# pymc-devs/pymc

Measured on AMD Instinct MI355X. Metric: effective samples/sec (and leapfrog steps/sec), 10k-param hierarchical logistic regression, one NUTS chain per GPU, higher is better.
Workload: dtype f64

## Files before the change

include/nuts_mi355.h:

```cpp
#ifndef NUTS_MI355_H
#define NUTS_MI355_H

#include <stdint.h>

#ifdef __cplusplus
extern "C" {
#endif

#define NUTS_OK 0
#define NUTS_E_BAD_ENERGY 1
#define NUTS_E_ARG 2
#define NUTS_E_HIP 3
#define NUTS_E_LINALG 4
#define NUTS_E_CALLBACK 5


enum { NUTS_TR_NONE = 0, NUTS_TR_LOG = 1, NUTS_TR_LOGODDS = 2, NUTS_TR_INTERVAL = 3 };
enum {
  NUTS_OP_CONST = 0, NUTS_OP_DATA = 1, NUTS_OP_VAR = 2,
  NUTS_OP_TMP = 3,
  NUTS_OP_GATHER = 4,
  NUTS_OP_LIN = 5
};
enum {
// ... 122 lines not shown
  const double *glm_X;
  const double *glm_y;
  int32_t n_lins, pad3;
  const nuts_lin *lins;
} nuts_model_spec;
enum { NUTS_GLM_NORMAL = 0, NUTS_GLM_BERNOULLI = 1, NUTS_GLM_POISSON = 2 };
#define NUTS_GLM_MAXP 512

typedef struct nuts_model nuts_model;
typedef struct nuts_chain nuts_chain;

int nuts_set_option(const char *name, int32_t value);
int nuts_unset_option(const char *name);
void nuts_clear_options(void);

int nuts_device_count(void);
int nuts_set_device(int device);
const char *nuts_last_error(void);

nuts_model *nuts_model_create(const nuts_model_spec *spec);
void nuts_model_destroy(nuts_model *m);
int32_t nuts_model_ndim(const nuts_model *m);
int nuts_model_logp_grad(nuts_model *m, const double *q, double *logp, double *grad);
int nuts_model_time_logp_grad(nuts_model *m, const double *q, int reps, double *ms_total, double *ms_dominant);
int nuts_model_debug_ticks(nuts_model *m, int64_t *out );
int64_t nuts_model_algorithmic_bytes(const nuts_model *m);
int nuts_model_get_scalar(const nuts_model *m, const char *name, double *out);

enum { NUTS_POT_DIAG_ADAPT = 0, NUTS_POT_DIAG = 1, NUTS_POT_FULL = 2,
       NUTS_POT_DIAG_ADAPT_EXP = 3,
// ... 168 lines not shown
```

pymc_amd/_lib.py:

```python

from __future__ import annotations

import ctypes as C
import os
import threading

import numpy as np

_HERE = os.path.dirname(os.path.abspath(__file__))
LIB_PATH = os.path.join(_HERE, "libnuts_mi355.so")

NUTS_OK, NUTS_E_BAD_ENERGY, NUTS_E_ARG, NUTS_E_HIP, NUTS_E_LINALG, NUTS_E_CALLBACK = 0, 1, 2, 3, 4, 5


class EngineError(RuntimeError):
    """A HIP/runtime failure inside libnuts_mi355 (maps to ParallelSamplingError-style reporting)."""


class Operand(C.Structure):
    _fields_ = [("kind", C.c_int32), ("ref", C.c_int32), ("c", C.c_double)]


class Term(C.Structure):
    _fields_ = [("a", Operand), ("b", Operand), ("c", Operand)]
# ... 222 lines not shown
    "nuts_chain_set_log_step_bar": (C.c_int, [_VP, C.c_double, C.c_double]),
    "nuts_gibbs_plan": (C.c_int, [C.POINTER(Pcg64), C.c_int64, C.c_int32, _VP, _VP, _VP, _PD]),
    "nuts_gibbs_plan_shuffle": (C.c_int, [C.POINTER(Pcg64), C.c_int64, _VP]),
    "nuts_gibbs_plan_draws": (C.c_int, [C.POINTER(Pcg64), C.c_int64, _VP, _VP, _VP, _PD, C.POINTER(C.c_int32)]),
    "nuts_gibbs_plan_skip": (C.c_int, [C.POINTER(Pcg64), C.c_int64, C.c_int32]),
    "nuts_gibbs_create": (_VP, [C.c_int64, C.c_int32, _PD]),
    "nuts_gibbs_destroy": (None, [_VP]),
    "nuts_gibbs_stage_slots": (C.c_int, []),
    "nuts_gibbs_stage": (C.c_int, [_VP, C.c_int32, _VP, _VP, _PD]),
    "nuts_gibbs_sweep_staged": (C.c_int, [_VP, C.c_int32, _VP, _VP, C.c_int32, _PD, _PD, _PD, C.POINTER(C.c_int64), C.POINTER(C.c_int64), _PD, _PD, _PD]),
    "nuts_gibbs_sweep": (C.c_int, [_VP, _VP, _PD, _PD, _PD, _VP, _VP, _PD, C.POINTER(C.c_int64), C.POINTER(C.c_int64), _PD, _PD, _PD]),
    "nuts_gibbs_plan_doubles": (C.c_int, [C.POINTER(Pcg64), C.c_int64, C.c_int32, _VP, C.c_int64, _PD]),
    "nuts_gibbs_sweep_prop": (C.c_int, [_VP, _VP, _VP, _PD, _PD, _PD, _VP, _PD, _PD, _VP, C.POINTER(C.c_int64), _PD, _PD, _PD]),
    "nuts_set_option": (C.c_int, [C.c_char_p, C.c_int32]),
    "nuts_clear_options": (None, []),
    "nuts_advi_create": (_VP, [C.POINTER(AdviConfig)]),
    "nuts_advi_destroy": (None, [_VP]),
    "nuts_advi_steps": (C.c_int, [_VP, C.c_int32, _VP, _PD, _PD]),
    "nuts_advi_get_params": (C.c_int, [_VP, _PD, _PD]),
    "nuts_advi_set_params": (C.c_int, [_VP, _PD, _PD]),
    "nuts_chain_profile": (C.c_int, [_VP, C.c_int]),
    "nuts_chain_profile_read": (C.c_int, [_VP, _PD, C.POINTER(C.c_int64), C.POINTER(C.c_int64)]),
    "nuts_group_create": (_VP, []),
    "nuts_group_add": (C.c_int, [_VP, _VP]),
    "nuts_group_remove": (C.c_int, [_VP, _VP]),
    "nuts_group_destroy": (None, [_VP]),
    "nuts_group_launches": (C.c_int, [_VP, C.POINTER(C.c_int64)]),
    "nuts_group_launches_wide": (C.c_int, [_VP, C.POINTER(C.c_int64), C.POINTER(C.c_int32)]),
    "nuts_unset_option": (C.c_int, [C.c_char_p]),
}
# ... 102 lines not shown
```

pymc_amd/csrc/engine.hip:

```cpp
#include <hip/hip_runtime.h>

#include <algorithm>
#include <atomic>
#include <chrono>
#include <cmath>
#include <cstdio>
#include <cstdlib>
#include <cstring>
#include <mutex>
#include <thread>
#include <utility>
#include <ctime>
#include <string>
#include <vector>

#include "kernels.h"
#include "small_kernel.h"
#include "mixture_kernel.h"
#include "nuts_mi355.h"
#include "pcg64_stream.h"
#include "advi.h"

static thread_local std::string g_err;

// ... 29 lines not shown
}

template <typename T>
static T* dev_alloc(size_t count) {
  void* p = nullptr;
  const size_t bytes = std::max<size_t>(count, 1) * sizeof(T);
  if (hipMalloc(&p, bytes) != hipSuccess) return nullptr;
  if (env_int("NUTS_POISON_ALLOC", 0)) { hipMemset(p, 0xFF, bytes); hipDeviceSynchronize(); }
  return static_cast<T*>(p);
}
template <typename T>
static T* dev_upload(const T* src, size_t count) {
  T* p = dev_alloc<T>(count);
  if (p && count) hipMemcpy(p, src, count * sizeof(T), hipMemcpyHostToDevice);
  return p;
}

#define PROF_RUN_MIN 16
#define SMALL_MAX_ELEMS 16384
#define SMALL_MAX_N 1024

struct nuts_model {
  ModelDev md{};
  hipStream_t stream = nullptr;
  std::vector<void*> owned;
  double* q_dev = nullptr;
  double* g_dev = nullptr;
  double* lp_dev = nullptr;
  double* host_pin = nullptr;
  std::vector<nuts_data_ref> data_refs;
// ... 13 lines not shown
  std::vector<int32_t> ev_units;
  int run_open = 0;
  int64_t runs_seen = 0;
  size_t ev_used = 0;
  int64_t dom_launches = 0;
  int sample_every = 1;
  hipStream_t own_stream = nullptr;
  struct nuts_group* group = nullptr;
  bool g_active = false;
  int gslot = 0;
  int n_chains = 0;
  int64_t pool_extra = 0;
  int64_t orphan_elems = 0, factor_elems = 0;
  double rows_pack_s = 0.0;
  int64_t rows_xt_len = 0, rows_y_len = 0;
  std::vector<LinDev> lins_host;

  template <typename T>
  T* keep(T* p) {
    owned.push_back((void*)p);
    return p;
  }
};

extern "C" int nuts_device_count(void) {
  int n = 0;
  if (hipGetDeviceCount(&n) != hipSuccess) return 0;
  return n;
}
extern "C" int nuts_set_device(int device) {
// ... 352 lines not shown
    if (prof) { hipEventRecord(m->ev[m->ev_used + 1], m->stream); m->ev_used += 2; m->dom_units += 1; }
    m->dom_launches++;
    hipLaunchKernelGGL(k_glm_reduce, dim3((md.glm.Ppad + 3 + GLM_RED_COLS - 1) / GLM_RED_COLS), dim3(GLM_RED_CHUNKS * GLM_RED_COLS), 0, m->stream, md, A, io, j);
    if (!md.has_mvn) return;
    prof = false; m->dom_launches--;
  }
  if (md.has_logit && md.lg.ga) {
    const int rev = m->rows_alternate ? (m->rows_flip ^= 1) : 0;
    const int par = (m->ga_par ^= 1);
    const dim3 grid(m->rows_grid + (fold ? 1 : 0) + md.lg.ga_naux), block(WAVE * md.lg.ga_w);
    GaArgs ga{md, A, io, j, rev, fold ? (GA_FOLD_CTL | GA_FOLD_SRC) : 0, par, d, max_depth, Emax, st, io, j - 1, d, 0, 0};
    if (fold && job) {
      ga.fold = GA_FOLD_CTL | (job->src_prev ? GA_FOLD_SRC : 0);
      ga.cio = job->io; ga.cj = job->j; ga.cd = job->d; ga.cseq = job->seq;
    }
    if (m->group && m->g_active && io.mode == MODE_TREE && m->group->kind >= 2) {
      GaLeafArgs L;
      L.A = A; L.io = io; L.cio = ga.cio; L.Emax = Emax; L.st = st;
      L.ga_part = md.lg.ga_part; L.ga_bpart = md.lg.ga_bpart; L.ga_ticket = md.lg.ga_ticket; L.def_loc = md.def_loc;
      L.j = j; L.fold = ga.fold; L.par = par; L.d = d; L.max_depth = max_depth; L.cj = ga.cj; L.cd = ga.cd; L.cseq = ga.cseq;
      L.slot = m->gslot; L.pad = 0;
      group_deposit(m, L);
    } else
    if (md.lg.ga_gpw) {
      switch (md.lg.D) {
        case 8: if (md.lg.ga_dx == 7) hipLaunchKernelGGL((k_rows_gb<8, 7>), grid, block, 0, m->stream, ga);
                else hipLaunchKernelGGL((k_rows_gb<8>), grid, block, 0, m->stream, ga); break;
        case 4: hipLaunchKernelGGL((k_rows_gb<4>), grid, block, 0, m->stream, ga); break;
        case 2: hipLaunchKernelGGL((k_rows_gb<2>), grid, block, 0, m->stream, ga); break;
        case 1: hipLaunchKernelGGL((k_rows_gb<1>), grid, block, 0, m->stream, ga); break;
// ... 799 lines not shown
      lg.Xp = m->keep(dev_upload(xp.data(), xp.size()));
      lg.ga_pcoff = m->keep(dev_upload(pcoff.data(), pcoff.size()));
      lg.ga_pexc_idx = m->keep(dev_upload(exc_idx.data(), exc_idx.size()));
      lg.ga_pexc = m->keep(dev_upload(exc.data(), exc.size()));
      lg.ga_pack_ebase20 = (uint32_t)plan.elo << 20;
      lg.ga_pack = (lg.Xp && lg.ga_pcoff && lg.ga_pexc_idx && lg.ga_pexc) ? 1 : 0;
      if (!lg.ga_pack) (void)hipGetLastError();
    }
    m->rows_pack_s = std::chrono::duration<double>(std::chrono::steady_clock::now() - t0).count();
  }
  lg.ga_coff = m->keep(dev_upload(coff.data(), coff.size()));
  lg.ga_tile0 = m->keep(dev_upload(tile0.data(), tile0.size()));
  lg.ga_part = m->keep(dev_alloc<double>((size_t)lg.G * PART_STRIDE));
  const size_t bpart_len = gpw ? 2 * (size_t)PART_STRIDE * ((lg.ga_nrec + WAVE - 1) / WAVE * WAVE) : 2 * (size_t)lg.ga_nrec * PART_STRIDE;
  lg.ga_bpart = m->keep(dev_alloc<double>(bpart_len));
  lg.ga_ticket = m->keep(dev_alloc<unsigned>(lg.ga_nblk));
  if (lg.ga_part) hipMemset(lg.ga_part, 0, (size_t)lg.G * PART_STRIDE * sizeof(double));
  if (lg.ga_bpart) hipMemset(lg.ga_bpart, 0, bpart_len * sizeof(double));
  if (lg.ga_ticket) hipMemset(lg.ga_ticket, 0, lg.ga_nblk * sizeof(unsigned));
  m->rows_grid = gpw ? lg.ga_nblk : lg.G;
  return true;
}

static bool build_rows_spans(nuts_model* m, const nuts_model_spec* s, int cus) {
  RowsDev& lg = m->md.lg;
  const int D = lg.D, SPAN = WAVE * m->rows_rpl;
  const int32_t* gid = s->rows_gid;
  int wpc = env_int("NUTS_ROWS_WAVES_PER_CU", 0);
  if (wpc <= 0) {
    const int64_t spans = (s->rows_N + (int64_t)WAVE * m->rows_rpl - 1) / ((int64_t)WAVE * m->rows_rpl);
    wpc = spans >= (int64_t)cus * 32 * 4 ? 32 : 16;
  }
  {
    std::vector<double> xt((size_t)D * lg.Npad, 0.0);
// ... 460 lines not shown
extern "C" int nuts_model_debug_ticks(nuts_model* m, int64_t* out) {
  if (!m || !out) return NUTS_E_ARG;
  HIPCHK(hipStreamSynchronize(m->stream));
  HIPCHK(hipMemcpy(out, m->md.ticks, 64 * sizeof(long long), hipMemcpyDeviceToHost));
  return NUTS_OK;
}

extern "C" int32_t nuts_model_ndim(const nuts_model* m) { return m ? m->md.n : -1; }
extern "C" int nuts_model_get_scalar(const nuts_model* m, const char* name, double* out) {
  if (!m || !name || !out) return NUTS_E_ARG;
  const std::string k(name);
  if (k == "rows_group_aligned") *out = m->md.lg.ga;
  else if (k == "rows_group_block") *out = m->md.lg.ga_gpw;
  else if (k == "rows_packed") *out = m->md.lg.ga ? m->md.lg.ga_pack : 0;
  else if (k == "rows_pack_build_s") *out = m->rows_pack_s;
  else if (k == "rows_aux_workgroups") *out = m->md.lg.ga ? m->md.lg.ga_naux : 0;
  else if (k == "mixture_workgroups") *out = m->md.has_mix ? m->md.mix.nwg : 0;
  else if (k == "glm_workgroups") *out = m->md.has_glm ? m->md.glm.nwg : 0;
  else if (k == "glm_row_stride") *out = m->md.has_glm ? m->md.glm.xstride : 0;
  else if (k == "glm_layout_width") *out = m->md.has_glm ? m->md.glm.Ppad : 0;
  else if (k == "mvn_row_aligned") *out = m->md.has_mvn ? m->md.mv.aligned : 0;
  else if (k == "rows_waves") *out = m->md.lg.ga ? m->md.lg.ga_w : m->md.lg.n_waves;
  else if (k == "lean") *out = m->md.lean_ok;
  else if (k == "chain_group_kind") {
    const RowsDev& lg = m->md.lg;
    const bool is_mvn = m->md.has_mvn && (m->md.mv.aligned == 4 || m->md.mv.aligned == 8 || m->md.mv.aligned == 16);
    const bool is_rows = m->md.has_logit && !m->md.has_mvn && lg.ga && lg.ga_naux == 0 && lg.D == 8 && m->ga_struct_ok == 1;
    *out = is_mvn ? 1.0 : (is_rows ? (lg.ga_gpw > 0 ? 3.0 : 2.0) : 0.0);
  }
  else if (k == "chain_group_wide_ok") *out = (m->md.has_mvn && m->md.mv.aligned > 0 && m->md.mv.k % 16 == 0) ? 1.0 : 0.0;
// ... 176 lines not shown
  std::vector<double> div_source, div_dest;
  bool cache_ok = false;
  std::vector<double> last_q;
  double last_logp = 0.0;
  DrawOut* do_dev = nullptr;
  DrawOut* do_host = nullptr;
  DrawOutMapped* dom_host = nullptr;
  DrawOutMapped* dom_dev = nullptr;
  unsigned dom_seq = 0;
  double* kin_part = nullptr;
  int64_t cache_epoch = -1;
  int fold_ctl = 1;
  CtlJob pend{}; bool pend_valid = false;
  bool defer_last_ctl = false; int xfold = 1;
  int next_dir = 0; bool pre_done = false; int xpre = 1;
  int spec_max = 10, last_depth = 0;
  int pipe_draws = 1;
  int logs_done = 0, logs_total = 0;
  double* many_in_host = nullptr; double* many_in_dev = nullptr; char* many_out_host = nullptr; char* many_out_dev = nullptr;
  size_t many_in_cap = 0, many_out_cap = 0;
  double t_begin = 0, t_loop = 0, t_wait = 0, t_finish = 0, t_post = 0;
  double tm_pre = 0, tm_start = 0, tm_tree = 0, tm_record = 0, tm_host = 0, tm_post = 0;
  int64_t tm_draws = 0, tm_batches = 0;
  int64_t leapfrogs = 0;
  int n_uni_cap = 0;
  template <typename T>
  T* keep(T* p) { owned.push_back((void*)p); return p; }
};

extern "C" void nuts_chain_config_default(nuts_chain_config* c) {
// ... 134 lines not shown
  A.S = 1 << maxd;
  A.ept = m->ept;
  A.nblk = m->md.nblk;
  const size_t arena = (size_t)A.S * n;
  A.Q = c->keep(dev_alloc<double>(arena)); A.P = c->keep(dev_alloc<double>(arena));
  A.V = c->keep(dev_alloc<double>(arena)); A.G = c->keep(dev_alloc<double>(arena));
  A.E = c->keep(dev_alloc<double>(A.S)); A.LOGP = c->keep(dev_alloc<double>(A.S));
  A.PS = c->keep(dev_alloc<double>((size_t)MAX_LEVELS * n));
  A.PSUM = c->keep(dev_alloc<double>(n));
  c->kin_part = c->keep(dev_alloc<double>((size_t)A.nblk));
  A.ctl = c->keep(dev_alloc<Ctl>(1));
  c->var = c->keep(dev_alloc<double>(n)); c->stds = c->keep(dev_alloc<double>(n)); c->inv_stds = c->keep(dev_alloc<double>(n));
  c->wa_mean = c->keep(dev_alloc<double>(n)); c->wa_m2 = c->keep(dev_alloc<double>(n));
  c->wb_mean = c->keep(dev_alloc<double>(n)); c->wb_m2 = c->keep(dev_alloc<double>(n));
  A.var = c->var; A.inv_stds = c->inv_stds;
  A.ga_ticket = m->md.lg.ga ? m->md.lg.ga_ticket : nullptr; A.ga_nticket = m->md.lg.ga ? m->md.lg.ga_nblk : 0;
  if (c->full_adapt) {
    const size_t nn = (size_t)n * n;
    c->fa_initial_cov.assign(cfg->dense_cov, cfg->dense_cov + nn);
    c->dense_C = c->keep(dev_alloc<double>(nn));
    c->fa_L = c->keep(dev_alloc<double>(nn)); c->fa_Lw = c->keep(dev_alloc<double>(nn));
    c->fa_fg_raw = c->keep(dev_alloc<double>(nn)); c->fa_bg_raw = c->keep(dev_alloc<double>(nn));
    c->fa_fg_mean = c->keep(dev_alloc<double>(n)); c->fa_bg_mean = c->keep(dev_alloc<double>(n));
    c->fa_scratch = c->keep(dev_alloc<double>(4 * (size_t)n)); c->fa_rhs = c->keep(dev_alloc<double>(n));
    c->fa_fail = c->keep(dev_alloc<int>(2));
    c->mv_grid = (n + (256 / WAVE) - 1) / (256 / WAVE);
  } else if (c->host_pot) {
    c->hp_p.assign(n, 0.0); c->hp_v.assign(n, 0.0);
    c->kin_user_dev = c->keep(dev_alloc<double>(1));
    A.kin_user = c->kin_user_dev;
  } else if (c->dense) {
    c->dense_C = c->keep(dev_upload(cfg->dense_cov, (size_t)n * n));
    c->dense_W = c->keep(dev_upload(cfg->dense_rand, (size_t)n * n));
    c->mv_grid = (n + (256 / WAVE) - 1) / (256 / WAVE);
  }
  c->n_uni_cap = (1 << maxd) + 2 * maxd + 16;
  c->stage_dev = c->keep(dev_alloc<double>(2 * (size_t)n + 2 * (size_t)c->n_uni_cap));
  c->out_dev = c->keep(dev_alloc<double>(2 * (size_t)n));
  c->out_dev2 = c->keep(dev_alloc<double>(2 * (size_t)n + 2));
  c->fold_ctl = env_int("NUTS_FOLD_CTL", 1) != 0 && !(m->md.has_mvn && m->md.mv.winv);
  c->spec_max = env_int("NUTS_SPEC_MAX", 10);
  c->xfold = env_int("NUTS_XFOLD", 1);
  c->pipe_draws = env_int("NUTS_PIPE_DRAWS", 1) != 0;
  c->xpre = env_int("NUTS_XPRE", 1);
  c->small_lds_slots = env_int("NUTS_SMALL_LDS", 1) == 0 ? -1 : env_int("NUTS_SMALL_LDS_SLOTS", 0);
  c->small_one_wave = env_int("NUTS_SMALL_ONE_WAVE", 1);
  c->group_wide = env_int("NUTS_GROUP_WIDE", 0);
  const bool glm_small = m->md.has_glm && env_int("NUTS_GLM_SMALL", 1) != 0 && m->md.glm.Xt && !m->md.glm.beta_buf && m->md.glm.off_beta >= 0 && m->md.n_derived == 0 && n <= 256;
  c->small = env_int("NUTS_SMALL_KERNEL", 1) != 0 && n <= SMALL_MAX_N && m->ept == 1 && !m->md.has_logit && !m->md.has_mvn && !m->md.has_mix &&
             (!m->md.has_glm || glm_small) &&
             m->md.n_lins == 0 && m->factor_elems <= SMALL_MAX_ELEMS && !c->dense;
  c->do_dev = c->keep(dev_alloc<DrawOut>(1));
  A.uniforms = c->stage_dev + 2 * (size_t)n;
  A.log_uniforms = A.uniforms + c->n_uni_cap;
  for (void* p : c->owned)
    if (!p) { g_err = "device allocation failed (trajectory arena needs 4*2^max_treedepth*n*8 bytes)"; nuts_chain_destroy(c); return nullptr; }
  if (hipHostMalloc((void**)&c->stage_host, (2 * (size_t)n + 2 * (size_t)c->n_uni_cap) * sizeof(double), hipHostMallocDefault) != hipSuccess ||
// ... 541 lines not shown
  int rc = NUTS_OK;
  bool exhausted = true;
  GroupTreeScope lockstep(c->dense || c->host_pot ? nullptr : c->m);
  unsigned flags = 0;
  Geometry gm{uniforms[0] < 0.5 ? 1 : -1, 0, 0, 0, 0.0};
  gm.eps = gm.dir > 0 ? step_size : -step_size;
  auto next_geometry = [&](const Geometry& g, int d, int dir) {
    Geometry r = g;
    if (g.dir > 0) r.right += 1 << d; else r.left -= 1 << d;
    r.dir = dir;
    r.edge = dir > 0 ? r.right : r.left;
    r.eps = dir > 0 ? step_size : -step_size;
    return r;
  };
  const int spec = c->host_pot ? 0 : std::min(c->spec_max, c->last_depth - 1);
  auto enqueue_doubling = [&](const Geometry& g, int d) {
    const int nleaf = 1 << d;
    ensure_logs(c, (2 << d) + d + 1);
    const int seq = ++c->seq;
    c->defer_last_ctl = c->xfold && c->fold_ctl && d + 1 < max_depth && d + 1 <= spec;
    c->next_dir = c->defer_last_ctl ? (uniforms[(2 << d) + d] < 0.5 ? 1 : -1) : 0;
    for (int j = 0; j < nleaf; ++j) enqueue_leaf(c, g, j, d, MODE_TREE, max_depth, j + 1 == nleaf ? seq : 0);
    c->defer_last_ctl = false;
    return seq;
  };
  c->pre_done = false;
  c->pend_valid = false;
  auto flush_pending = [&](int seq_waited) {
    if (!c->pend_valid || c->pend.seq != seq_waited) return;
    const CtlJob& p = c->pend;
    launch_control_lean(c->m, c->A, p.io, p.j, p.d, c->cfg.Emax, max_depth, c->st_dev, p.seq);
    c->pend_valid = false;
  };
  Geometry ahead{};
  int ahead_seq = 0;
  int seq = enqueue_doubling(gm, 0);
  int depth_done = 0;
// ... 1 lines not shown
    if (d + 1 < max_depth && d + 1 <= spec) {
      ahead = next_geometry(gm, d, uniforms[(2 << d) + d] < 0.5 ? 1 : -1);
      ahead_seq = enqueue_doubling(ahead, d + 1);
    } else ahead_seq = 0;
    flush_pending(seq);
    if (c->cb_err) return host_pot_error(c);
    const auto tw0 = clk::now();
    rc = wait_status(c, seq, &flags, cursor_out);
    c->t_wait += secs(tw0, clk::now());
    if (rc) return rc;
    depth_done = d + 1;
    if (flags & ST_BAD_ENERGY) break;
    if (flags & (ST_DIVERGING | ST_TURNING)) { exhausted = false; break; }
    if (d + 1 >= max_depth) break;
    const int dir = (flags & ST_DIR_POS) ? 1 : -1;
    if (ahead_seq) {
      if (ahead.dir != dir) { g_err = "internal error: look-ahead mispredicted the direction of a doubling"; return NUTS_E_HIP; }
      gm = ahead; seq = ahead_seq;
    } else {
      gm = next_geometry(gm, d, dir);
      seq = enqueue_doubling(gm, d + 1);
    }
  }
  c->last_depth = depth_done;
  c->pend_valid = false;
  *flags_out = flags;
  *exhausted_out = exhausted;
  return NUTS_OK;
}

static void launch_small(nuts_chain* c, const ArenaDev& A, const SmallDrawArgs& a) {
#define SMALL_LAUNCH(NT, P) hipLaunchKernelGGL((k_small_draw<NT, P>), dim3(1), dim3(NT), 0, c->m->stream, c->m->md, A, a)
  const bool hp = c->m->has_prog;
  if (c->n <= WAVE && c->small_one_wave && !c->m->md.has_glm) { if (hp) SMALL_LAUNCH(64, true); else SMALL_LAUNCH(64, false); }
  else if (c->n <= 256) { if (hp) SMALL_LAUNCH(256, true); else SMALL_LAUNCH(256, false); }
  else if (c->n <= 512) { if (hp) SMALL_LAUNCH(512, true); else SMALL_LAUNCH(512, false); }
  else { if (hp) SMALL_LAUNCH(1024, true); else SMALL_LAUNCH(1024, false); }
#undef SMALL_LAUNCH
}

// ... 1123 lines not shown
```

pymc_amd/csrc/rows_ga_kernel.h:

```cpp
#pragma once
#include "rows_kernel.h"
#include "rows_pack.h"

__device__ __forceinline__ void ga_def_local(const RowsDev& R, bool is_mu, double qn, double& gx, double& dxdq, double& dj, double& lp) {
  if (is_mu) {
    const double r = qn - R.mu_c[0];
    const double z = r * R.mu_c[1];
    lp = -0.5 * z * z - R.mu_c[2] + (-0.91893853320467274178);
    gx = -z * R.mu_c[1]; dxdq = 1.0; dj = 0.0;
  } else {
    double x, lj;
    if (R.sigma_tr == NUTS_TR_LOG) { x = exp(qn); dxdq = x; lj = qn; dj = 1.0; }
    else { x = qn; dxdq = 1.0; lj = 0.0; dj = 0.0; }
    const double z = x * R.sg_c[0];
    double lpf = -0.5 * z * z - R.sg_c[1] + (-0.22579135264472743236);
    double g = -z * R.sg_c[0];
    if (!(x >= 0)) { lpf = -INFINITY; g = 0.0; }
    gx = g; lp = lj + lpf;
  }
}

template <int D, int RPL>
__device__ __forceinline__ void ga_load(const RowsDev& R, int64_t xoff, int lane, double (&x)[D][RPL], uint32_t& ybits) {
  constexpr int SPAN = WAVE * RPL;
// ... 186 lines not shown
    for (int d = 0; d < D; ++d) eta = fma(x[d][k], beta[d], eta);
    double l, rr;
    logit_row(eta, (double)((yb >> (8 * k)) & 0xffu), l, rr);
    const bool in = lane * RPL + k < nvalid;
    lp += in ? l : 0.0;
    rr = in ? rr : 0.0;
#pragma unroll
    for (int d = 0; d < D; ++d) acc[d] = fma(rr, x[d][k], acc[d]);
    if constexpr (!ILV) __builtin_amdgcn_sched_barrier(0);
  }
}

#define GA_MAXW 4
#define GA_MAXCHUNK 8
#define GA_F_NOTAIL 1

struct GaArgs;
template <int D>
__device__ __forceinline__ void ga_tail(const GaArgs& T, int g, double (&s_acc)[4][2][D + 1], double (&s_red)[NDOT],
                                        double (&s_cp)[8][PART_STRIDE], int (&s_info)[4], double (&s_keep)[5][WAVE]);

struct GaArgs {
  ModelDev md; ArenaDev A; EvalIO io;
  int j, rev, fold, par, d, max_depth;
  double Emax;
  HostStatus* st;
  EvalIO cio;
  int cj, cd, cseq, cpad;
};
#define GA_FOLD_CTL 1
// ... 352 lines not shown
  const bool tree = io.mode == MODE_TREE;
  const int dl = lane % D;
  const int iz = R.off_z + g * D + dl;
  MergePrefetch mpf;
  if (w == 0 && tree && !(R.ga_flags & GA_F_NOTAIL)) merge_prefetch(A, lf, j, iz, mpf);
  __syncthreads();
  if (R.ga_flags & GA_F_NOTAIL) return;

  if (w == 0)
    ga_tail_wave<D, false>(R, A, io, R.ga_part, R.ga_ticket, md.def_loc, lf, g, W, j, T.par, T.d, s_acc, s_red, s_info,
                           s_keep[0][lane], s_keep[1][lane], s_keep[2][lane], s_keep[3][lane], s_keep[4][lane], &mpf);
  __syncthreads();
  if (!s_info[0]) return;
  ga_block_partial<D>(R, R.ga_part, R.ga_bpart, T.par, g, leaf, s_info, s_cp);
}
```

pymc_amd/csrc/rows_ga_multi_kernel.h:

```cpp
#pragma once
#include "mvn_multi_kernel.h"

#define GAM_MAXC 8
#define GAM_MAXNC 4

struct GaLeafArgs {
  ArenaDev A;
  EvalIO io, cio;
  double Emax;
  HostStatus* st;
  double* ga_part;
  double* ga_bpart;
  unsigned* ga_ticket;
  double* def_loc;
  int j, fold, par, d, max_depth, cj, cd, cseq;
  int slot, pad;
};

template <int NC>
struct GaMultiArgs {
  GaLeafArgs c[NC];
  int rev, pad;
};

__device__ __forceinline__ LeanSrc gam_src(const RowsDev& R, const GaLeafArgs& L, int par) {
  return LeanSrc{L.ga_bpart + (int64_t)par * R.ga_nrec * PART_STRIDE, PART_STRIDE, R.ga_nrec, L.def_loc + (int64_t)par * 4 * MAX_DEFERRED};
}

template <int DX>
__device__ __forceinline__ void gam_load(const double* base , const int8_t* ybase, int lane,
                                         typename GaTileSel<DX>::type& t) {
  const ga_v2d* p = reinterpret_cast<const ga_v2d*>(base) + lane;
#pragma unroll
  for (int k = 0; k < DX; ++k) t.c[k] = p[k * WAVE];
  t.y = *reinterpret_cast<const uint16_t*>(ybase + 2 * lane);
}

template <int NC, int OCC, int DX>
__global__ __launch_bounds__(64 * GA_MAXW, OCC) void k_rows_ga_multi(ModelDev md, GaMultiArgs<NC> ma) {
  constexpr int D = 8, RPL = 2, SPAN = WAVE * RPL, PIPE = 2;
  typedef typename GaTileSel<DX>::type Tile;
  const RowsDev& R = md.lg;
  if ((int)blockIdx.x < GAM_MAXC) {
    int ci = -1;
#pragma unroll
    for (int c = 0; c < NC; ++c) ci = (int)blockIdx.x == ma.c[c].slot ? c : ci;
    if (ci < 0) return;
    const GaLeafArgs& L = ma.c[ci];
    if (L.fold & GA_FOLD_CTL) control_lean(md, L.A, L.cio, L.cj, L.cd, L.Emax, L.max_depth, L.st, L.cseq, gam_src(R, L, L.par ^ 1));
    return;
  }
  const int g = (int)blockIdx.x - GAM_MAXC;
  const int rev = ma.rev;
  const int tid = threadIdx.x, lane = tid & (WAVE - 1), w = __builtin_amdgcn_readfirstlane(tid >> 6), W = (int)blockDim.x >> 6;
  __shared__ double s_acc[NC][GA_MAXW][2][D + 1];
  __shared__ double s_red[NC][NDOT];
  __shared__ double s_cp[GA_MAXCHUNK][PART_STRIDE];
  __shared__ int s_info[NC][4];
  __shared__ double s_keep[NC][5][WAVE];
  __shared__ double s_beta[NC][D];
  __shared__ __attribute__((aligned(16))) char s_args[(sizeof(GaMultiArgs<NC>) + 15) / 16 * 16];

  int T; int64_t ng, cbase;
  if (R.ga_T_uni > 0) { T = R.ga_T_uni; ng = R.ga_ng_uni; cbase = (int64_t)(g * W + w) * R.ga_cstride_uni; }
  else {
    T = __builtin_amdgcn_readfirstlane(R.ga_tile0[g + 1] - R.ga_tile0[g]);
    ng = __builtin_amdgcn_readfirstlane((int)(R.gptr[g + 1] - R.gptr[g]));
    const int64_t cb = R.ga_coff[g * W + w];
    cbase = ((int64_t)__builtin_amdgcn_readfirstlane((int)(cb >> 32)) << 32) | (uint32_t)__builtin_amdgcn_readfirstlane((int)(cb & 0xffffffffll));
  }
  const int c0 = (int)((int64_t)w * T / W), c2 = (int)((int64_t)(w + 1) * T / W);
  const int n = c2 - c0;
  const int nA = (n + 1) / 2;
  const int nsw = rev ? n - nA : nA;
  constexpr int64_t TS = (int64_t)DX * SPAN;
  auto local_at = [&](int i) { return rev ? (i < nsw ? nA + i : i - nsw) : i; };
  auto tile_at = [&](int i) { return cbase + (int64_t)local_at(i) * TS; };
  const int l_last = (c2 == T) ? n - 1 : -1;
  const int n_last = (int)(ng - (int64_t)(T - 1) * SPAN);
  if (lane == 0) {
#pragma unroll
    for (int c = 0; c < NC; ++c)
#pragma unroll
      for (int dd = 0; dd <= D; ++dd) { s_acc[c][w][0][dd] = 0.0; s_acc[c][w][1][dd] = 0.0; }
  }
  {
    static_assert(alignof(GaMultiArgs<NC>) == 8 && sizeof(GaMultiArgs<NC>) % 8 == 0, "kernarg layout: the second argument follows the model at the next multiple of 8");
    const uint2* ka = (const uint2*)__builtin_amdgcn_kernarg_segment_ptr() + (sizeof(ModelDev) + 7) / 8;
    for (int t = tid; t < (int)(sizeof(GaMultiArgs<NC>) / 8); t += (int)blockDim.x) reinterpret_cast<uint2*>(s_args)[t] = ka[t];
  }

  int dead = 0;
#pragma unroll
  for (int c = 0; c < NC; ++c) dead |= load_aborted(ma.c[c].io, ma.c[c].A) ? (1 << c) : 0;
  if (dead == (1 << NC) - 1) return;
  for (int c = w; c < NC; c += W) {
    const GaLeafArgs& L = ma.c[c];
    Leaf lf; QView qv;
    resolve_leaf(L.io, L.A, L.j, lf, qv);
    double hval0, hph0;
    ga_hyper<D>(R, qv, L.fold, gam_src(R, L, L.par ^ 1), lane, hval0, hph0);
    const int dl = lane % D;
    const int iz = R.off_z + g * D + dl;
    double zq, zph, m_lane, s_lane;
    ga_z_state(qv, iz, zq, zph);
    ga_hyper_lanes<D>(R, hval0, dl, m_lane, s_lane);
    const double bl = fma(s_lane, zq, m_lane);
    if (lane < D) s_beta[c][lane] = bl;
    s_keep[c][0][lane] = hval0; s_keep[c][1][lane] = hph0; s_keep[c][2][lane] = zq; s_keep[c][3][lane] = zph; s_keep[c][4][lane] = s_lane;
  }
  __syncthreads();
  constexpr bool TWO = NC <= 3;
  Tile ta, tb;
  {
    const int64_t o0 = tile_at(0), o1 = tile_at(min(1, max(n - 1, 0)));
    gam_load<DX>(R.Xt + o0, R.y + o0 / DX, lane, ta);
// ... 57 lines not shown
        if (i + 1 >= n) break;
        issue(i + 2, ta);
        GAM_STAGE(tb, i + 1)
        issue(i + 3, tb);
      }
    } else {
      for (int i = 0; i < n; ++i) {
        GAM_STAGE(ta, i)
        issue(i + 1, ta);
      }
    }
#undef GAM_STAGE
    if (n > 0) flush();
  }

  const GaMultiArgs<NC>& Tm = *reinterpret_cast<const GaMultiArgs<NC>*>(s_args);
  MergePrefetch mpf;
  if (w < NC && !((dead >> w) & 1)) {
    const GaLeafArgs& L = Tm.c[w];
    Leaf lf; QView qv;
    resolve_leaf(L.io, L.A, L.j, lf, qv);
    merge_prefetch(L.A, lf, L.j, R.off_z + g * D + lane % D, mpf);
  }
  __syncthreads();
  for (int c = w; c < NC; c += W) {
    if ((dead >> c) & 1) { if (lane == 0) s_info[c][0] = 0; continue; }
    const GaLeafArgs& L = Tm.c[c];
    Leaf lf; QView qv;
    resolve_leaf(L.io, L.A, L.j, lf, qv);
    auto tail = [&](const MergePrefetch* pf) {
      ga_tail_wave<D, true>(R, L.A, L.io, L.ga_part, L.ga_ticket, L.def_loc, lf, g, W, L.j, L.par, L.d, s_acc[c], s_red[c], s_info[c],
                            s_keep[c][0][lane], s_keep[c][1][lane], s_keep[c][2][lane], s_keep[c][3][lane], s_keep[c][4][lane], pf);
    };
    if (c == w) tail(&mpf);
    else tail(nullptr);
  }
  __syncthreads();
#pragma unroll
  for (int c = 0; c < NC; ++c) {
    if (!s_info[c][0]) continue;
    ga_block_partial<D>(R, Tm.c[c].ga_part, Tm.c[c].ga_bpart, Tm.c[c].par, g, true, s_info[c], s_cp);
    __syncthreads();
  }
}
// ... 1 lines not shown
```

Baseline: 19160.

## Pair NUTS leaf evaluations with speculative opposite-direction shadow leaves via ring buffer

When the tree is expected to turn, each leaf evaluation also computes a speculative leaf on the opposite trajectory edge inside the same multi-leaf rows kernel. The shadow leaf's per-group partial sums go to a device ring buffer, and a later doubling in that direction replays them through a lighter tail-only kernel instead of streaming the design matrix again. The aim is to amortise X reads across two leaves per pass. The cost is extra ring, partial and shadow-state memory, wasted shadow work when the tree stops early, and more complex ticket and parity bookkeeping.

```diff
diff --git a/include/nuts_mi355.h b/include/nuts_mi355.h
--- a/include/nuts_mi355.h
+++ b/include/nuts_mi355.h
@@ -160,6 +160,9 @@
 int nuts_unset_option(const char *name);
 void nuts_clear_options(void);
 
+int64_t nuts_edge_pair_plan(const int32_t *dirs, int32_t n_dirs, int32_t n_doublings, int32_t spec, int32_t max_depth,
+                            int32_t ring, int32_t *out, int64_t out_cap);
+
 int nuts_device_count(void);
 int nuts_set_device(int device);
 const char *nuts_last_error(void);
diff --git a/pymc_amd/_lib.py b/pymc_amd/_lib.py
--- a/pymc_amd/_lib.py
+++ b/pymc_amd/_lib.py
@@ -260,6 +260,7 @@
     "nuts_gibbs_sweep_prop": (C.c_int, [_VP, _VP, _VP, _PD, _PD, _PD, _VP, _PD, _PD, _VP, C.POINTER(C.c_int64), _PD, _PD, _PD]),
     "nuts_set_option": (C.c_int, [C.c_char_p, C.c_int32]),
     "nuts_clear_options": (None, []),
+    "nuts_edge_pair_plan": (C.c_int64, [C.POINTER(C.c_int32), C.c_int32, C.c_int32, C.c_int32, C.c_int32, C.c_int32, C.POINTER(C.c_int32), C.c_int64]),
     "nuts_advi_create": (_VP, [C.POINTER(AdviConfig)]),
     "nuts_advi_destroy": (None, [_VP]),
     "nuts_advi_steps": (C.c_int, [_VP, C.c_int32, _VP, _PD, _PD]),
diff --git a/pymc_amd/csrc/engine.hip b/pymc_amd/csrc/engine.hip
--- a/pymc_amd/csrc/engine.hip
+++ b/pymc_amd/csrc/engine.hip
@@ -67,6 +67,48 @@
   T* p = dev_alloc<T>(count);
   if (p && count) hipMemcpy(p, src, count * sizeof(T), hipMemcpyHostToDevice);
   return p;
+}
+
+enum { EP_PLAIN = 0, EP_PAIRED = 1, EP_REPLAY = 2 };
+struct EdgePlan {
+  int ring = 64;
+  int side = 0, n = 0;
+  unsigned head = 0;
+  int cap = 0, used = 0;
+  int64_t ring_full = 0;
+  void reset() { side = 0; n = 0; cap = 0; used = 0; }
+  template <class F>
+  void begin(int d, int dir, int last, F dir_of) {
+    cap = 0; used = 0;
+    for (int e = d + 1; e <= last; ++e)
+      if (dir_of(e) == -dir) { cap = std::min(1 << std::min(e, 30), ring); break; }
+  }
+  int leaf(int dir, int* slot, int* k) {
+    if (n > 0 && side == dir) { *slot = (int)(head % (unsigned)ring); *k = used++; ++head; --n; return EP_REPLAY; }
+    if (cap > 0 && n < cap) { side = -dir; *k = n; *slot = (int)((head + (unsigned)n) % (unsigned)ring); ++n; return EP_PAIRED; }
+    if (cap > 0 && n >= ring) ++ring_full;
+    *slot = -1; *k = -1;
+    return EP_PLAIN;
+  }
+};
+extern "C" int64_t nuts_edge_pair_plan(const int32_t* dirs, int32_t n_dirs, int32_t n_doublings, int32_t spec, int32_t max_depth,
+                                       int32_t ring, int32_t* out, int64_t out_cap) {
+  if (!dirs || !out || n_doublings < 0 || n_doublings > n_dirs || n_doublings > 20 || ring < 1) { g_err = "nuts_edge_pair_plan: bad argument"; return -1; }
+  EdgePlan ep;
+  ep.ring = ring;
+  int64_t n = 0;
+  const int last = std::min(std::min(spec, max_depth - 1), n_dirs - 1);
+  for (int d = 0; d < n_doublings; ++d) {
+    ep.begin(d, dirs[d], last, [&](int e) { return (int)dirs[e]; });
+    for (int j = 0; j < (1 << d); ++j, ++n) {
+      int slot, k;
+      const int kind = ep.leaf(dirs[d], &slot, &k);
+      if (n >= out_cap) { g_err = "nuts_edge_pair_plan: output too small"; return -1; }
+      int32_t* o = out + 5 * n;
+      o[0] = d; o[1] = j; o[2] = kind; o[3] = slot; o[4] = k;
+    }
+  }
+  return n;
 }
 
 #define PROF_RUN_MIN 16
@@ -110,6 +152,16 @@
   int64_t orphan_elems = 0, factor_elems = 0;
   double rows_pack_s = 0.0;
   int64_t rows_xt_len = 0, rows_y_len = 0;
+  int ep_ok = 0, ep_par = 0;
+  double *ep_ring = nullptr, *ep_part = nullptr, *ep_bpart = nullptr, *ep_def_loc = nullptr;
+  int64_t ep_ring_bytes = 0, ep_shadows = 0, ep_replays = 0;
+  int64_t ep_dropped = 0;
+  int64_t ep_ring_full = 0;
+  int ep_turns = 0;
+  struct EpLaunch {
+    int kind = EP_PLAIN, slot = 0, sj = 0, sfold = 0, first = 0;
+    EvalIO sio{}; ArenaDev sA{};
+  } ep_launch;
   std::vector<LinDev> lins_host;
 
   template <typename T>
@@ -492,6 +544,32 @@
       ga.fold = GA_FOLD_CTL | (job->src_prev ? GA_FOLD_SRC : 0);
       ga.cio = job->io; ga.cj = job->j; ga.cd = job->d; ga.cseq = job->seq;
     }
+    const nuts_model::EpLaunch ep = m->ep_launch;
+    m->ep_launch.kind = EP_PLAIN;
+    if (ep.kind == EP_PAIRED) {
+      GaMultiArgs<2, true> ma;
+      GaLeafArgs& L = ma.c[0];
+      L.A = A; L.io = io; L.cio = ga.cio; L.Emax = Emax; L.st = st;
+      L.ga_part = md.lg.ga_part; L.ga_bpart = md.lg.ga_bpart; L.ga_ticket = md.lg.ga_ticket; L.def_loc = md.def_loc;
+      L.j = j; L.fold = ga.fold; L.par = par; L.d = d; L.max_depth = max_depth; L.cj = ga.cj; L.cd = ga.cd; L.cseq = ga.cseq;
+      L.slot = 0; L.pad = 0;
+      GaLeafArgs& S = ma.c[1];
+      S.A = ep.sA; S.io = ep.sio; S.cio = ep.sio; S.Emax = Emax; S.st = nullptr;
+      S.ga_part = m->ep_part; S.ga_bpart = m->ep_bpart; S.ga_ticket = md.lg.ga_ticket + md.lg.ga_nblk; S.def_loc = m->ep_def_loc;
+      S.j = ep.sj; S.fold = ep.sfold; S.par = (m->ep_par ^= 1); S.d = 0; S.max_depth = 1; S.cj = 0; S.cd = 0; S.cseq = 0;
+      S.slot = GAM_MAXC - 1; S.pad = ep.first ? GAM_SH_FIRST : 0;
+      ma.rev = rev; ma.pad = 0;
+      ma.ring = m->ep_ring + (size_t)ep.slot * md.lg.G * GA_RING_DOUBLES(8);
+      const dim3 pgrid(GAM_MAXC + md.lg.G);
+      if (md.lg.ga_dx == 7) hipLaunchKernelGGL((k_rows_ga_multi<2, 3, 7, true>), pgrid, block, 0, m->stream, md, ma);
+      else hipLaunchKernelGGL((k_rows_ga_multi<2, 3, 8, true>), pgrid, block, 0, m->stream, md, ma);
+      m->ep_shadows++;
+    } else if (ep.kind == EP_REPLAY) {
+      const dim3 rgrid(m->rows_grid + (fold ? 1 : 0));
+      hipLaunchKernelGGL((k_rows_ga_replay<8>), rgrid, block, 0, m->stream, ga,
+                         (const double*)(m->ep_ring + (size_t)ep.slot * md.lg.G * GA_RING_DOUBLES(8)));
+      m->ep_replays++;
+    } else
     if (m->group && m->g_active && io.mode == MODE_TREE && m->group->kind >= 2) {
       GaLeafArgs L;
       L.A = A; L.io = io; L.cio = ga.cio; L.Emax = Emax; L.st = st;
@@ -1321,10 +1399,24 @@
   lg.ga_part = m->keep(dev_alloc<double>((size_t)lg.G * PART_STRIDE));
   const size_t bpart_len = gpw ? 2 * (size_t)PART_STRIDE * ((lg.ga_nrec + WAVE - 1) / WAVE * WAVE) : 2 * (size_t)lg.ga_nrec * PART_STRIDE;
   lg.ga_bpart = m->keep(dev_alloc<double>(bpart_len));
-  lg.ga_ticket = m->keep(dev_alloc<unsigned>(lg.ga_nblk));
+  lg.ga_ticket = m->keep(dev_alloc<unsigned>(2 * (size_t)lg.ga_nblk));
   if (lg.ga_part) hipMemset(lg.ga_part, 0, (size_t)lg.G * PART_STRIDE * sizeof(double));
   if (lg.ga_bpart) hipMemset(lg.ga_bpart, 0, bpart_len * sizeof(double));
-  if (lg.ga_ticket) hipMemset(lg.ga_ticket, 0, lg.ga_nblk * sizeof(unsigned));
+  if (lg.ga_ticket) hipMemset(lg.ga_ticket, 0, 2 * (size_t)lg.ga_nblk * sizeof(unsigned));
+  m->ep_ok = 0;
+  if (!gpw && D == 8 && m->rows_rpl == 2 && m->ga_struct_ok == 1 && lg.ga_naux == 0 && env_int("NUTS_EDGE_PAIR", 1) != 0) {
+    const size_t ring_len = (size_t)GA_RING_LEAVES * lg.G * GA_RING_DOUBLES(8);
+    m->ep_ring = m->keep(dev_alloc<double>(ring_len));
+    m->ep_part = m->keep(dev_alloc<double>((size_t)lg.G * PART_STRIDE));
+    m->ep_bpart = m->keep(dev_alloc<double>(bpart_len));
+    m->ep_def_loc = m->keep(dev_alloc<double>(2 * 4 * (size_t)MAX_DEFERRED));
+    if (m->ep_ring && m->ep_part && m->ep_bpart && m->ep_def_loc) {
+      hipMemset(m->ep_part, 0, (size_t)lg.G * PART_STRIDE * sizeof(double));
+      hipMemset(m->ep_bpart, 0, bpart_len * sizeof(double));
+      hipMemset(m->ep_def_loc, 0, 2 * 4 * (size_t)MAX_DEFERRED * sizeof(double));
+      m->ep_ok = 1; m->ep_ring_bytes = (int64_t)(ring_len * sizeof(double));
+    } else (void)hipGetLastError();
+  }
   m->rows_grid = gpw ? lg.ga_nblk : lg.G;
   return true;
 }
@@ -1815,6 +1907,13 @@
   else if (k == "rows_group_block") *out = m->md.lg.ga_gpw;
   else if (k == "rows_packed") *out = m->md.lg.ga ? m->md.lg.ga_pack : 0;
   else if (k == "rows_pack_build_s") *out = m->rows_pack_s;
+  else if (k == "edge_pair") *out = m->ep_ok;
+  else if (k == "edge_pair_ring_bytes") *out = (double)m->ep_ring_bytes;
+  else if (k == "edge_pair_shadows") *out = (double)m->ep_shadows;
+  else if (k == "edge_pair_replays") *out = (double)m->ep_replays;
+  else if (k == "edge_pair_turns") *out = m->ep_turns;
+  else if (k == "edge_pair_dropped") *out = (double)m->ep_dropped;
+  else if (k == "edge_pair_ring_full") *out = (double)m->ep_ring_full;
   else if (k == "rows_aux_workgroups") *out = m->md.lg.ga ? m->md.lg.ga_naux : 0;
   else if (k == "mixture_workgroups") *out = m->md.has_mix ? m->md.mix.nwg : 0;
   else if (k == "glm_workgroups") *out = m->md.has_glm ? m->md.glm.nwg : 0;
@@ -2021,6 +2120,9 @@
   CtlJob pend{}; bool pend_valid = false;
   bool defer_last_ctl = false; int xfold = 1;
   int next_dir = 0; bool pre_done = false; int xpre = 1;
+  bool edge_pair = false;
+  ArenaDev shA{};
+  EdgePlan ep;
   int spec_max = 10, last_depth = 0;
   int pipe_draws = 1;
   int logs_done = 0, logs_total = 0;
@@ -2185,7 +2287,7 @@
   c->wa_mean = c->keep(dev_alloc<double>(n)); c->wa_m2 = c->keep(dev_alloc<double>(n));
   c->wb_mean = c->keep(dev_alloc<double>(n)); c->wb_m2 = c->keep(dev_alloc<double>(n));
   A.var = c->var; A.inv_stds = c->inv_stds;
-  A.ga_ticket = m->md.lg.ga ? m->md.lg.ga_ticket : nullptr; A.ga_nticket = m->md.lg.ga ? m->md.lg.ga_nblk : 0;
+  A.ga_ticket = m->md.lg.ga ? m->md.lg.ga_ticket : nullptr; A.ga_nticket = m->md.lg.ga ? 2 * m->md.lg.ga_nblk : 0;
   if (c->full_adapt) {
     const size_t nn = (size_t)n * n;
     c->fa_initial_cov.assign(cfg->dense_cov, cfg->dense_cov + nn);
@@ -2212,6 +2314,16 @@
   c->fold_ctl = env_int("NUTS_FOLD_CTL", 1) != 0 && !(m->md.has_mvn && m->md.mv.winv);
   c->spec_max = env_int("NUTS_SPEC_MAX", 10);
   c->xfold = env_int("NUTS_XFOLD", 1);
+  c->edge_pair = m->ep_ok && env_int("NUTS_EDGE_PAIR", 1) != 0 && !c->dense && !c->host_pot && !m->md.has_mvn && !m->explicit_pre &&
+                 m->md.lean_ok && c->fold_ctl && c->xfold;
+  if (c->edge_pair) {
+    c->shA = A;
+    c->shA.S = 2;
+    c->shA.Q = c->keep(dev_alloc<double>(2 * (size_t)n)); c->shA.P = c->keep(dev_alloc<double>(2 * (size_t)n));
+    c->shA.V = c->keep(dev_alloc<double>(2 * (size_t)n)); c->shA.G = c->keep(dev_alloc<double>(2 * (size_t)n));
+    if (!c->shA.Q || !c->shA.P || !c->shA.V || !c->shA.G) { (void)hipGetLastError(); c->edge_pair = false; }
+    c->ep.ring = std::max(1, std::min(GA_RING_LEAVES, env_int("NUTS_EDGE_PAIR_RING", GA_RING_LEAVES)));
+  }
   c->pipe_draws = env_int("NUTS_PIPE_DRAWS", 1) != 0;
   c->xpre = env_int("NUTS_XPRE", 1);
   c->small_lds_slots = env_int("NUTS_SMALL_LDS", 1) == 0 ? -1 : env_int("NUTS_SMALL_LDS_SLOTS", 0);
@@ -2783,13 +2895,41 @@
     return r;
   };
   const int spec = c->host_pot ? 0 : std::min(c->spec_max, c->last_depth - 1);
+  const bool pairing = c->edge_pair && !c->m->group && !c->host_pot && !c->dense;
+  int turns = 0;
+  int ep_replays_in[32] = {};
+  int prev_dir = 0;
+  bool ep_bad = false;
+  c->ep.reset();
+  c->m->ep_launch.kind = EP_PLAIN;
   auto enqueue_doubling = [&](const Geometry& g, int d) {
     const int nleaf = 1 << d;
     ensure_logs(c, (2 << d) + d + 1);
     const int seq = ++c->seq;
     c->defer_last_ctl = c->xfold && c->fold_ctl && d + 1 < max_depth && d + 1 <= spec;
     c->next_dir = c->defer_last_ctl ? (uniforms[(2 << d) + d] < 0.5 ? 1 : -1) : 0;
-    for (int j = 0; j < nleaf; ++j) enqueue_leaf(c, g, j, d, MODE_TREE, max_depth, j + 1 == nleaf ? seq : 0);
+    if (pairing) c->ep.begin(d, g.dir, std::min(spec, max_depth - 1), [&](int e) { return uniforms[(1 << e) + e - 1] < 0.5 ? 1 : -1; });
+    for (int j = 0; j < nleaf; ++j) {
+      if (pairing) {
+        nuts_model::EpLaunch& el = c->m->ep_launch;
+        int k = 0;
+        el.kind = c->ep.leaf(g.dir, &el.slot, &k);
+        if (el.kind == EP_REPLAY) ++ep_replays_in[std::min(d, 31)];
+        if (el.kind == EP_REPLAY && k != j) { g_err = "internal error: edge pairing replays a leaf out of order"; ep_bad = true; el.kind = EP_PLAIN; }
+        if (el.kind == EP_PAIRED) {
+          const int od = -g.dir;
+          EvalIO sio{};
+          sio.mode = MODE_SIMPLE; sio.lean = 1;
+          sio.dir = od; sio.edge = od > 0 ? g.right : g.left; sio.left = g.left; sio.right = g.right;
+          sio.eps = od > 0 ? step_size : -step_size;
+          el.sio = sio; el.sj = k; el.sA = c->shA;
+          el.first = k == 0;
+          el.sfold = k > 0 ? GA_FOLD_SRC : (j == 0 && d > 0 && prev_dir == od ? GA_FOLD_SRC : 0);
+        }
+      }
+      enqueue_leaf(c, g, j, d, MODE_TREE, max_depth, j + 1 == nleaf ? seq : 0);
+    }
+    prev_dir = g.dir;
     c->defer_last_ctl = false;
     return seq;
   };
@@ -2821,6 +2961,7 @@
     if (flags & (ST_DIVERGING | ST_TURNING)) { exhausted = false; break; }
     if (d + 1 >= max_depth) break;
     const int dir = (flags & ST_DIR_POS) ? 1 : -1;
+    turns += dir != gm.dir;
     if (ahead_seq) {
       if (ahead.dir != dir) { g_err = "internal error: look-ahead mispredicted the direction of a doubling"; return NUTS_E_HIP; }
       gm = ahead; seq = ahead_seq;
@@ -2831,6 +2972,13 @@
   }
   c->last_depth = depth_done;
   c->pend_valid = false;
+  if (depth_done >= 4) c->m->ep_turns = std::max(c->m->ep_turns, turns);
+  c->m->ep_ring_full = c->ep.ring_full;
+  if (pairing) {
+    c->m->ep_dropped += c->ep.n;
+    for (int d = depth_done; d < 32; ++d) c->m->ep_dropped += ep_replays_in[d];
+  }
+  if (ep_bad) return NUTS_E_HIP;
   *flags_out = flags;
   *exhausted_out = exhausted;
   return NUTS_OK;
diff --git a/pymc_amd/csrc/rows_ga_kernel.h b/pymc_amd/csrc/rows_ga_kernel.h
--- a/pymc_amd/csrc/rows_ga_kernel.h
+++ b/pymc_amd/csrc/rows_ga_kernel.h
@@ -224,6 +224,8 @@
 #define GA_MAXW 4
 #define GA_MAXCHUNK 8
 #define GA_F_NOTAIL 1
+#define GA_RING_LEAVES 64
+#define GA_RING_DOUBLES(D) (GA_MAXW * 2 * ((D) + 1))
 
 struct GaArgs;
 template <int D>
@@ -606,3 +608,51 @@
   if (!s_info[0]) return;
   ga_block_partial<D>(R, R.ga_part, R.ga_bpart, T.par, g, leaf, s_info, s_cp);
 }
+
+template <int D>
+__global__ __launch_bounds__(64 * GA_MAXW, 4) void k_rows_ga_replay(GaArgs a, const double* __restrict__ ring) {
+  const ModelDev& md = a.md;
+  const ArenaDev& A = a.A;
+  const EvalIO& io = a.io;
+  const int fold = a.fold, par = a.par;
+  const RowsDev& R = md.lg;
+  int b = (int)blockIdx.x;
+  if (fold & GA_FOLD_CTL) {
+    if (b == 0) { control_lean(md, A, a.cio, a.cj, a.cd, a.Emax, a.max_depth, a.st, a.cseq, lean_src(md, par ^ 1)); return; }
+    --b;
+  }
+  const int g = b;
+  if (g >= R.G) return;
+  const int tid = threadIdx.x, lane = tid & (WAVE - 1), w = __builtin_amdgcn_readfirstlane(tid >> 6);
+  Leaf lf; QView qv;
+  const int aborted = load_aborted(io, A);
+  resolve_leaf(io, A, a.j, lf, qv);
+  __shared__ double s_acc[GA_MAXW][2][D + 1];
+  __shared__ double s_red[NDOT];
+  __shared__ double s_cp[GA_MAXCHUNK][PART_STRIDE];
+  __shared__ int s_info[4];
+  __shared__ double s_keep[5][WAVE];
+  __shared__ __attribute__((aligned(16))) char s_args[(sizeof(GaArgs) + 15) / 16 * 16];
+  constexpr int NR = GA_RING_DOUBLES(D);
+  static_assert(NR <= 2 * WAVE, "two doubles of a ring entry per thread at most");
+  const double rv0 = ring[(int64_t)g * NR + min(tid, NR - 1)], rv1 = ring[(int64_t)g * NR + min(tid + WAVE, NR - 1)];
+  {
+    const uint4* ka = (const uint4*)__builtin_amdgcn_kernarg_segment_ptr();
+    for (int t = tid; t < (int)((sizeof(GaArgs) + 15) / 16); t += (int)blockDim.x) reinterpret_cast<uint4*>(s_args)[t] = ka[t];
+  }
+  __syncthreads();
+  if (w == 0) {
+    double hval0, hph0, zq, zph, m_lane, s_lane;
+    ga_hyper<D>(R, qv, fold, lean_src(md, par ^ 1), lane, hval0, hph0);
+    const int dl = lane % D;
+    ga_z_state(qv, R.off_z + g * D + dl, zq, zph);
+    ga_hyper_lanes<D>(R, hval0, dl, m_lane, s_lane);
+    s_keep[0][lane] = hval0; s_keep[1][lane] = hph0; s_keep[2][lane] = zq; s_keep[3][lane] = zph; s_keep[4][lane] = s_lane;
+  }
+  if (aborted) return;
+  if (tid < WAVE) {
+    (&s_acc[0][0][0])[tid] = rv0;
+    if (tid + WAVE < NR) (&s_acc[0][0][0])[tid + WAVE] = rv1;
+  }
+  ga_tail<D>(*reinterpret_cast<const GaArgs*>(s_args), g, s_acc, s_red, s_cp, s_info, s_keep);
+}
diff --git a/pymc_amd/csrc/rows_ga_multi_kernel.h b/pymc_amd/csrc/rows_ga_multi_kernel.h
--- a/pymc_amd/csrc/rows_ga_multi_kernel.h
+++ b/pymc_amd/csrc/rows_ga_multi_kernel.h
@@ -17,11 +17,18 @@
   int slot, pad;
 };
 
-template <int NC>
+template <int NC, bool SH = false>
 struct GaMultiArgs {
   GaLeafArgs c[NC];
   int rev, pad;
 };
+#define GAM_SH_FIRST 1
+template <int NC>
+struct GaMultiArgs<NC, true> {
+  GaLeafArgs c[NC];
+  int rev, pad;
+  double* ring;
+};
 
 __device__ __forceinline__ LeanSrc gam_src(const RowsDev& R, const GaLeafArgs& L, int par) {
   return LeanSrc{L.ga_bpart + (int64_t)par * R.ga_nrec * PART_STRIDE, PART_STRIDE, R.ga_nrec, L.def_loc + (int64_t)par * 4 * MAX_DEFERRED};
@@ -36,9 +43,11 @@
   t.y = *reinterpret_cast<const uint16_t*>(ybase + 2 * lane);
 }
 
-template <int NC, int OCC, int DX>
-__global__ __launch_bounds__(64 * GA_MAXW, OCC) void k_rows_ga_multi(ModelDev md, GaMultiArgs<NC> ma) {
+template <int NC, int OCC, int DX, bool SH = false>
+__global__ __launch_bounds__(64 * GA_MAXW, OCC) void k_rows_ga_multi(ModelDev md, GaMultiArgs<NC, SH> ma) {
   constexpr int D = 8, RPL = 2, SPAN = WAVE * RPL, PIPE = 2;
+  static_assert(!SH || NC == 2, "edge pairing: the chain's leaf and one shadow leaf");
+  typedef GaMultiArgs<NC, SH> Args;
   typedef typename GaTileSel<DX>::type Tile;
   const RowsDev& R = md.lg;
   if ((int)blockIdx.x < GAM_MAXC) {
@@ -59,7 +68,7 @@
   __shared__ int s_info[NC][4];
   __shared__ double s_keep[NC][5][WAVE];
   __shared__ double s_beta[NC][D];
-  __shared__ __attribute__((aligned(16))) char s_args[(sizeof(GaMultiArgs<NC>) + 15) / 16 * 16];
+  __shared__ __attribute__((aligned(16))) char s_args[(sizeof(Args) + 15) / 16 * 16];
 
   int T; int64_t ng, cbase;
   if (R.ga_T_uni > 0) { T = R.ga_T_uni; ng = R.ga_ng_uni; cbase = (int64_t)(g * W + w) * R.ga_cstride_uni; }
@@ -85,21 +94,27 @@
       for (int dd = 0; dd <= D; ++dd) { s_acc[c][w][0][dd] = 0.0; s_acc[c][w][1][dd] = 0.0; }
   }
   {
-    static_assert(alignof(GaMultiArgs<NC>) == 8 && sizeof(GaMultiArgs<NC>) % 8 == 0, "kernarg layout: the second argument follows the model at the next multiple of 8");
+    static_assert(alignof(Args) == 8 && sizeof(Args) % 8 == 0, "kernarg layout: the second argument follows the model at the next multiple of 8");
     const uint2* ka = (const uint2*)__builtin_amdgcn_kernarg_segment_ptr() + (sizeof(ModelDev) + 7) / 8;
-    for (int t = tid; t < (int)(sizeof(GaMultiArgs<NC>) / 8); t += (int)blockDim.x) reinterpret_cast<uint2*>(s_args)[t] = ka[t];
+    for (int t = tid; t < (int)(sizeof(Args) / 8); t += (int)blockDim.x) reinterpret_cast<uint2*>(s_args)[t] = ka[t];
   }
 
   int dead = 0;
 #pragma unroll
   for (int c = 0; c < NC; ++c) dead |= load_aborted(ma.c[c].io, ma.c[c].A) ? (1 << c) : 0;
+  if constexpr (SH) dead = (dead & 1) ? 3 : 0;
   if (dead == (1 << NC) - 1) return;
   for (int c = w; c < NC; c += W) {
     const GaLeafArgs& L = ma.c[c];
     Leaf lf; QView qv;
-    resolve_leaf(L.io, L.A, L.j, lf, qv);
     double hval0, hph0;
-    ga_hyper<D>(R, qv, L.fold, gam_src(R, L, L.par ^ 1), lane, hval0, hph0);
+    if (SH && c == 1 && (L.pad & GAM_SH_FIRST)) {
+      resolve_leaf(L.io, ma.c[0].A, L.j, lf, qv);
+      ga_hyper<D>(R, qv, L.fold, gam_src(R, ma.c[0], ma.c[0].par ^ 1), lane, hval0, hph0);
+    } else {
+      resolve_leaf(L.io, L.A, L.j, lf, qv);
+      ga_hyper<D>(R, qv, L.fold, gam_src(R, L, L.par ^ 1), lane, hval0, hph0);
+    }
     const int dl = lane % D;
     const int iz = R.off_z + g * D + dl;
     double zq, zph, m_lane, s_lane;
@@ -187,20 +202,29 @@
     if (n > 0) flush();
   }
 
-  const GaMultiArgs<NC>& Tm = *reinterpret_cast<const GaMultiArgs<NC>*>(s_args);
+  const Args& Tm = *reinterpret_cast<const Args*>(s_args);
   MergePrefetch mpf;
-  if (w < NC && !((dead >> w) & 1)) {
+  if (w < NC && !((dead >> w) & 1) && !(SH && w == 1)) {
     const GaLeafArgs& L = Tm.c[w];
     Leaf lf; QView qv;
     resolve_leaf(L.io, L.A, L.j, lf, qv);
     merge_prefetch(L.A, lf, L.j, R.off_z + g * D + lane % D, mpf);
   }
   __syncthreads();
+  if constexpr (SH) {
+    constexpr int NR = GA_RING_DOUBLES(D);
+    for (int t = tid; t < NR; t += (int)blockDim.x) Tm.ring[(int64_t)g * NR + t] = (&s_acc[1][0][0][0])[t];
+  }
   for (int c = w; c < NC; c += W) {
     if ((dead >> c) & 1) { if (lane == 0) s_info[c][0] = 0; continue; }
     const GaLeafArgs& L = Tm.c[c];
     Leaf lf; QView qv;
     resolve_leaf(L.io, L.A, L.j, lf, qv);
+    if (SH && c == 1) {
+      ga_tail_wave<D, false>(R, L.A, L.io, L.ga_part, L.ga_ticket, L.def_loc, lf, g, W, L.j, L.par, L.d, s_acc[c], s_red[c], s_info[c],
+                             s_keep[c][0][lane], s_keep[c][1][lane], s_keep[c][2][lane], s_keep[c][3][lane], s_keep[c][4][lane], nullptr);
+      continue;
+    }
     auto tail = [&](const MergePrefetch* pf) {
       ga_tail_wave<D, true>(R, L.A, L.io, L.ga_part, L.ga_ticket, L.def_loc, lf, g, W, L.j, L.par, L.d, s_acc[c], s_red[c], s_info[c],
                             s_keep[c][0][lane], s_keep[c][1][lane], s_keep[c][2][lane], s_keep[c][3][lane], s_keep[c][4][lane], pf);
```

Result: faster. 20310, median of 6 (+6.0%).
